# jeremy-rifkin/Markov-Huffman-Coding

Hardware: AMD Instinct MI355X
Metric: encode+decode GB/s on 16 GB byte stream, bit-exact round-trip (higher is better)
Workload: dtype u8

## Files before the change

markov-huffman-coding_amd/csrc/mh_encode.hip:

```cpp
#include "mh_dev.hpp"

namespace mhk {


constexpr uint32_t O2H_MAP_OFF = 256, O2H_HOT_OFF = 256 + 64 * 64 * 2;
__device__ __forceinline__ void o2hot_lookup16(const unsigned char *img, const uint4 &x4, uint32_t ctx, uint32_t (&e)[16]) {
    const uint16_t *ctxmap = reinterpret_cast<const uint16_t *>(img + O2H_MAP_OFF);
    const uint16_t *hot = reinterpret_cast<const uint16_t *>(img + O2H_HOT_OFF);
    const uint32_t x[4] = {x4.x, x4.y, x4.z, x4.w};
    uint32_t id[18];
    id[0] = img[ctx >> 8];
    id[1] = img[ctx & 255u];
#pragma unroll
    for (int j = 0; j < 16; ++j) id[2 + j] = img[(x[j >> 2] >> (8 * (j & 3))) & 255u];
    uint32_t cs[16];
#pragma unroll
    for (int j = 0; j < 16; ++j) cs[j] = ctxmap[(id[j] << 6) | (id[j + 1] ^ id[j])];
#pragma unroll
    for (int j = 0; j < 16; ++j) e[j] = hot[(cs[j] << 6) | (id[j + 2] ^ id[j + 1])];
}

__device__ __forceinline__ void o2hot_lookup8(const unsigned char *img, uint32_t xa, uint32_t xb, uint32_t ctx, uint32_t (&e)[8]) {
    const uint16_t *ctxmap = reinterpret_cast<const uint16_t *>(img + O2H_MAP_OFF);
    const uint16_t *hot = reinterpret_cast<const uint16_t *>(img + O2H_HOT_OFF);
// ... 533 lines not shown
                }
                if (lane == 0) {
                    const uint64_t gend = base + total;
                    __hip_atomic_store(&cp.state[group], CH_PFX | (gend & CH_VAL), __ATOMIC_RELAXED, __HIP_MEMORY_SCOPE_AGENT);
                    if ((group + 1) * E_WAVES >= p.nwt) *cp.nbits = gend;
                    if (bad) atomicExch(cp.status, MHK_STATUS_TIMEOUT);
                    s_done[par] = 0;
                    s_base[par] = base;
                    s_bad[par] = bad ? 1u : 0u;
                    __hip_atomic_store(&s_tag[par], tag, __ATOMIC_RELEASE, __HIP_MEMORY_SCOPE_WORKGROUP);
                }
            }
            uint32_t spins = 0;
            const bool follower_hook = cp.probe == 3u && group != 0 && arrived != uint32_t(E_WAVES) - 1u;
            while (__hip_atomic_load(&s_tag[par], __ATOMIC_ACQUIRE, __HIP_MEMORY_SCOPE_WORKGROUP) != tag) {
                if (++spins > CH_SPIN_MAX * 8u || follower_hook) {
                    waited_out = true;
                    if (lane == 0) atomicExch(cp.status, MHK_STATUS_TIMEOUT);
                    break;
                }
                __builtin_amdgcn_s_sleep(1);
            }
            if (follower_hook && !waited_out) {
                waited_out = true;
                if (lane == 0) atomicExch(cp.status, MHK_STATUS_TIMEOUT);
            }
            uint64_t mine = lane < wave ? s_tile[par][lane] : 0ull;
#pragma unroll
            for (int d = 8; d >= 1; d >>= 1) mine += __shfl_xor(mine, d);
            s = s_base[par] + __shfl(mine, 0);
            if (s_bad[par]) waited_out = true;
        }
        if (wt < p.nwt) {
            const uint64_t end = s + tile_bits;
            if (lane == 0 && !waited_out && end > cap_bits) atomicExch(cp.status, MHK_STATUS_CAPACITY);
            emit = !(waited_out || end > cap_bits);
        }
        if (waited_out) break;
        const uint64_t wt_now = wt;
        __syncthreads();
        if (threadIdx.x == 0) s_ticket = atomicAdd(cp.sync, 1u);
        __syncthreads();
        group = s_ticket;
        wt = group * E_WAVES + wave;
        ahead = load_raw2(p.data, p.n, wt * E_WT + lane * E_VEC, p.prev0);
        if (emit) {
            uint64_t gbase = s >> 5;
            uint32_t cur = uint32_t(s & 31u);
            uint64_t abs_bits = s;
            uint32_t seam0 = (cur != 0 && wt_now != 0) ? SEAM_DROP : SEAM_NONE;
#pragma unroll 1
            for (int k = 0; k < E_SUBSTEPS; ++k) {
                const uint64_t off = wt_now * E_WT + uint64_t(k) * E_SUB + lane * E_VEC;
                const uint32_t nvalid = off + E_VEC <= p.n ? uint32_t(E_VEC) : off < p.n ? uint32_t(p.n - off) : 0u;
                uint32_t sub_bits;
                if ((escmask >> k) & 1u) {
                    const LaneIn again = load_raw2(p.data, p.n, off, p.prev0);
                    emit_substep_slow<2>(p, nullptr, stage, out32, again.x, h0.pb, nvalid, lane, off, abs_bits, gbase, cur, seam0, sub_bits);
                } else {
                    const uint32_t L = (h0.gl & 255u) + ((h0.gl >> 8) & 255u) + ((h0.gl >> 16) & 255u) + (h0.gl >> 24);
                    const uint32_t inc = wave_inclusive_sum(L);
                    sub_bits = __builtin_amdgcn_readlane(inc, 63);
                    const uint32_t exc = inc - L;
                    if (p.index && nvalid && ((uint32_t(off) & (S - 1u)) == 0u))
                        p.index[off >> p.chunk_shift] = (uint64_t(h0.pb) << 48) | (abs_bits + exc);
                    fine2_entry(p, S, lane, off, nvalid, h0.pb, exc);
                    uint32_t o = cur + exc;
#pragma unroll
                    for (int q = 0; q < 4; ++q) {
                        const uint32_t glq = (h0.gl >> (8 * q)) & 255u;
                        if (glq) deposit<false>(stage, h0.g[q] << (64u - glq), o, 0, 0);
                        o += glq;
                    }
                    const uint32_t nfull = (cur + sub_bits) >> 5;
                    flush_words(stage, out32, gbase, nfull, seam0, lane);
                    if (nfull) seam0 = SEAM_NONE;
                    gbase += nfull;
                    cur = (cur + sub_bits) & 31u;
                }
                abs_bits += sub_bits;
                h0 = h1; h1 = h2; h2 = h3;
            }
            if (cur != 0 && seam0 == SEAM_NONE) {
                const uint64_t next = (wt_now + 1) * uint64_t(E_WT);
                const uint64_t pos = next + lane;
                const bool valid = lane < 32u && pos < p.n;
                uint32_t l = 0;
                uint64_t c = 0;
                if (valid) o2_code_of(p, smem, p.data[pos - 2], p.data[pos - 1], p.data[pos], l, c);
                const uint32_t inc = wave_inclusive_sum(l);
                const uint32_t exc = inc - l;
                if (l && exc < 32u - cur) deposit<true>(stage, c << (64u - l), cur + exc, 0u, 1u);
                if (lane == 0) {
                    out32[gbase] = __builtin_bswap32(stage[0]);
                    stage[0] = 0;
                }
            } else if (cur != 0 && lane == 0) {
                stage[0] = 0;
            }
        }
    }
}

constexpr int R_IMG_WORDS = ((163840 - 131072 - 128) / 4) & ~7;
constexpr int R_HALF_WORDS = R_IMG_WORDS / 2;
constexpr uint32_t R_HALF_CAP_BITS = uint32_t(R_HALF_WORDS - 8) * 32u;
static_assert(R_IMG_WORDS >= E_WAVES * (E_STAGE_BITS / 32) + 16 && R_HALF_WORDS % 4 == 0, "image size");
constexpr int REGION_LDS_BYTES = 131072 + R_IMG_WORDS * 4 + 128;



__global__ __launch_bounds__(1024) void region_bits_kernel(const HistHeader *hdr, HistHeader expect, const uint32_t *slab,
                                                           const uint32_t *cross_all, const uint8_t *len8,
                                                           unsigned long long *region_bits, uint32_t *region_esc, int *status) {
    __shared__ unsigned long long part[16];
    __shared__ uint32_t any_esc;
    extern __shared__ __attribute__((aligned(16))) unsigned char lens[];
    for (uint32_t i = threadIdx.x; i < 65536u / 16u; i += 1024u) reinterpret_cast<uint4 *>(lens)[i] = reinterpret_cast<const uint4 *>(len8)[i];
    if (threadIdx.x == 0) any_esc = 0;
    __syncthreads();
    const uint32_t w = blockIdx.x, tid = threadIdx.x;
    if (hdr->magic != HIST_WS_MAGIC || hdr->n != expect.n || hdr->data != expect.data || hdr->region_vecs != expect.region_vecs ||
        hdr->grid != expect.grid || hdr->prev0 != expect.prev0 || hdr->cross_cap != expect.cross_cap) {
        if (tid == 0) { atomicExch(status, MHK_STATUS_CORRUPT); region_bits[w] = 0; region_esc[w] = 0; }
        return;
    }
    unsigned long long acc = 0;
    bool esc = false;
    const uint32_t *sl = slab + size_t(w) * 32768u;
    for (uint32_t i = tid; i < 32768u; i += 1024u) {
        const uint32_t v = sl[i];
        const uint32_t s0 = i, s1 = i | 0x8000u;
        const uint32_t l0 = lens[hist_slot_prev(s0) * 256u + (s0 >> 8)], l1 = lens[hist_slot_prev(s1) * 256u + (s1 >> 8)];
        acc += (unsigned long long)(v & 0xFFFFu) * l0;
        acc += (unsigned long long)(v >> 16) * l1;
        esc |= ((v & 0xFFFFu) && l0 > uint32_t(mh::ENC16_MAX_LEN)) || ((v >> 16) && l1 > uint32_t(mh::ENC16_MAX_LEN));
    }
    const uint32_t *cross = cross_all + size_t(w) * (expect.cross_cap + 1u);
    const uint32_t nc = cross[0];
    if (nc > expect.cross_cap && tid == 0) atomicExch(status, MHK_STATUS_CAPACITY);
    for (uint32_t i = tid; i < (nc < expect.cross_cap ? nc : expect.cross_cap); i += 1024u) {
        const uint32_t sl2 = cross[1u + i];
        const uint32_t l2 = lens[hist_slot_prev(sl2) * 256u + (sl2 >> 8)];
        acc += 16384ull * l2;
        esc |= l2 > uint32_t(mh::ENC16_MAX_LEN);
    }
    if (esc) atomicOr(&any_esc, 1u);
    for (int d = 32; d >= 1; d >>= 1) acc += __shfl_xor(acc, d);
    if ((tid & 63u) == 0) part[tid >> 6] = acc;
    __syncthreads();
    if (tid == 0) {
        unsigned long long t = 0;
        for (int i = 0; i < 16; ++i) t += part[i];
        region_bits[w] = t;
        region_esc[w] = any_esc;
    }
}

__global__ __launch_bounds__(SCAN_THREADS) void region_scan_kernel(const unsigned long long *region_bits, uint32_t nregion,
                                                                   unsigned long long *region_start, const unsigned long long *carry0,
                                                                   uint8_t *out, uint64_t cap, unsigned long long *nbits, int *status) {
    __shared__ uint64_t lds[SCAN_THREADS / 64];
    const uint64_t c0 = carry0 ? (*carry0 & 7ull) : 0;
    const uint32_t i = threadIdx.x;
    const uint64_t v = i < nregion ? region_bits[i] : 0;
    uint64_t total;
    const uint64_t ex = block_excl_scan(v, lds, total);
    const uint64_t s = c0 + ex;
    if (i < nregion) {
        region_start[i] = s;
        if (i > 0 && (s & 31u) && ((s >> 5) + 1) * 4 <= cap) reinterpret_cast<uint32_t *>(out)[s >> 5] = 0;
    }
    if (i == 0) {
        const uint64_t end = c0 + total;
        *nbits = end;
        if (end > cap * 8) atomicExch(status, MHK_STATUS_CAPACITY);
        const uint64_t endw = end >> 5;
        if ((end & 31u) && (endw + 1) * 4 <= cap) reinterpret_cast<uint32_t *>(out)[endw] = 0;
        else if (end & 31u) for (uint64_t b = endw * 4; b < cap; ++b) out[b] = 0;
        if ((c0 & 31u) && 4 <= cap) reinterpret_cast<uint32_t *>(out)[0] = 0;
    }
}

struct RegionParams {
    const unsigned long long *region_start;
    const unsigned long long *region_bits;
    const uint32_t *region_esc;
    uint64_t region_vecs;
    uint64_t nvec_up;
    uint64_t cap_words;
    int *status;
};
constexpr uint32_t R_IMG_CAP_BITS = E_WAVES * E_STAGE_BITS;

struct Roll1 {
    uint4 x; uint32_t prev;
    __device__ __forceinline__ uint32_t next_window() {
        const uint32_t sym = x.x & 255u;
        const uint32_t win = (sym << 8) | prev;
        prev = sym;
        x.x = __builtin_amdgcn_alignbyte(x.y, x.x, 1);
        x.y = __builtin_amdgcn_alignbyte(x.z, x.y, 1);
        x.z = __builtin_amdgcn_alignbyte(x.w, x.z, 1);
        x.w >>= 8;
        return win;
    }
};
__device__ __forceinline__ void code_of1(const uint8_t *len8, const uint64_t *code64, const uint16_t *tab, uint32_t win, bool valid, uint32_t &l, uint64_t &c) {
    const uint32_t e = valid ? uint32_t(tab[mh::enc_slot(win)]) : 0u;
    l = e >> 12;
    c = e & 0xFFFu;
    if (e >= 0xD000u) {
        const uint32_t nat = ((win & 255u) << 8) | (win >> 8);
        l = len8[nat];
        c = code64[nat];
        if (l > 64u) { l = 0; c = 0; }
    }
}
__device__ __forceinline__ uint32_t region_escape_bits(const uint8_t *len8, const uint64_t *code64, const uint16_t *tab, uint4 x, uint32_t pb, uint32_t nvalid) {
    Roll1 r{x, pb};
    uint32_t L = 0;
#pragma unroll 1
    for (uint32_t j = 0; j < 16; ++j) { uint32_t l; uint64_t c; code_of1(len8, code64, tab, r.next_window(), j < nvalid, l, c); L += l; }
    return L;
}
__device__ __forceinline__ void region_escape_deposit(const uint8_t *len8, const uint64_t *code64, const uint16_t *tab, uint32_t *img, uint4 x,
                                                   uint32_t pb, uint32_t nvalid, uint32_t o) {
    Roll1 r{x, pb};
#pragma unroll 1
    for (uint32_t j = 0; j < 16; ++j) {
        uint32_t l; uint64_t c;
        code_of1(len8, code64, tab, r.next_window(), j < nvalid, l, c);
        if (l) deposit<false>(img, c << (64u - l), o, 0, 0);
        o += l;
    }
}

__device__ __forceinline__ uint32_t region_round_lanes(uint64_t nsym, uint64_t bits) {
    const uint32_t cand[4] = {1024u, 1008u, 992u, 960u};
    uint32_t pick = 0;
#pragma unroll
    for (int c = 3; c >= 0; --c)
        if (bits * cand[c] * E_VEC * 201u <= uint64_t(R_HALF_CAP_BITS - 32u) * nsym * 200u) pick = cand[c];
    return pick ? pick : 1024u;
}

#ifdef MH_ENC_STAMP
#define ENC_STAMP(i) do { unsigned long long t_; __builtin_amdgcn_sched_barrier(0); \
        asm volatile("s_memtime %0\n\ts_waitcnt lgkmcnt(0)" : "=s"(t_) :: "memory"); __builtin_amdgcn_sched_barrier(0); \
        stamp_acc[i] += t_ - stamp_last; stamp_last = t_; } while (0)
#else
#define ENC_STAMP(i) do { } while (0)
#endif
template <bool ESCK, bool WIDE = false>
__global__ __launch_bounds__(E_THREADS) void enc_region_kernel(EmitParams p, RegionParams rp) {
    extern __shared__ __attribute__((aligned(16))) unsigned char smem[];
    if ((rp.region_esc[blockIdx.x] != 0) != ESCK) return;
    {
        const uint64_t v0 = uint64_t(blockIdx.x) * rp.region_vecs;
        const uint64_t v1 = v0 + rp.region_vecs < rp.nvec_up ? v0 + rp.region_vecs : rp.nvec_up;
        if (v0 < v1) {
            const uint32_t rs = ESCK ? uint32_t(E_THREADS) : region_round_lanes((v1 * E_VEC < p.n ? v1 * E_VEC : p.n) - v0 * E_VEC, rp.region_bits[blockIdx.x]);
            if ((rs != uint32_t(E_THREADS)) != WIDE) return;
        } else if (WIDE) return;
    }
    uint16_t *tab = reinterpret_cast<uint16_t *>(smem);
    uint32_t *img = reinterpret_cast<uint32_t *>(smem + 131072);
    uint32_t *sb = img + R_IMG_WORDS;
    const uint32_t tid = threadIdx.x, lane = tid & 63u, wave = tid >> 6;
    for (int i = tid; i < 8192; i += E_THREADS)
        reinterpret_cast<uint4 *>(tab)[i] = reinterpret_cast<const uint4 *>(p.enc16)[i];
    for (int i = tid; i < R_IMG_WORDS; i += E_THREADS) img[i] = 0;
    __syncthreads();
    if (*p.status != MHK_STATUS_OK) return;

    const uint64_t v0 = uint64_t(blockIdx.x) * rp.region_vecs;
    const uint64_t v1 = v0 + rp.region_vecs < rp.nvec_up ? v0 + rp.region_vecs : rp.nvec_up;
    if (v0 >= v1) return;
    uint32_t *out32 = reinterpret_cast<uint32_t *>(p.out);
    const uint32_t S = 1u << p.chunk_shift;
    const uint32_t RS = WIDE ? region_round_lanes((v1 * E_VEC < p.n ? v1 * E_VEC : p.n) - v0 * E_VEC, rp.region_bits[blockIdx.x]) : uint32_t(E_THREADS);
    const bool act = !WIDE || tid < RS;
    const bool wave_idles = WIDE && uint32_t(wave) * 64u + 63u >= RS;
    const uint64_t rounds = (v1 - v0 + RS - 1) / RS;
    const uint64_t s0 = rp.region_start[blockIdx.x];
    uint64_t gbase = s0 >> 5, abs_round = s0;
    uint32_t cur = uint32_t(s0 & 31u);
    bool seam_first = cur != 0;
    uint32_t carry = 0;
    bool prev_half = false;

    auto fetch = [&](uint64_t r) -> LaneIn {
        const uint64_t v = v0 + r * RS + tid;
        LaneIn in = load_raw(p.data, p.n, (act && v < v1) ? v * E_VEC : ~0ull >> 1, p.prev0);
        return in;
    };
    auto lookup16 = [&](const LaneIn &in, uint32_t pb, uint32_t (&e)[16]) {
        uint32_t w[16];
        slots16(in.x, pb, w);
#pragma unroll
        for (int j = 0; j < 16; ++j) e[j] = uint32_t(tab[w[j]]);
    };
    uint32_t *imgr = img;
    auto flush = [&](uint32_t nfull) -> uint32_t {
        uint32_t tail = 0;
        for (uint32_t j = tid * 4u; j <= nfull; j += E_THREADS * 4u) {
            const uint4 w = *reinterpret_cast<const uint4 *>(imgr + j);
            *reinterpret_cast<uint4 *>(imgr + j) = make_uint4(0, 0, 0, 0);
            const uint32_t v[4] = {__builtin_bswap32(w.x), __builtin_bswap32(w.y), __builtin_bswap32(w.z), __builtin_bswap32(w.w)};
            if (j + 4u <= nfull && !(j == 0 && seam_first) && gbase + j + 4u <= rp.cap_words) {
                struct __attribute__((packed, aligned(4))) Q4 { uint32_t a, b, c, d; };
                *reinterpret_cast<Q4 *>(out32 + gbase + j) = Q4{v[0], v[1], v[2], v[3]};
            } else {
#pragma unroll
                for (uint32_t k = 0; k < 4u; ++k) {
                    if (j + k >= nfull || gbase + j + k >= rp.cap_words) break;
                    if (j + k == 0 && seam_first) atomicOr(&out32[gbase], v[k]);
                    else out32[gbase + j + k] = v[k];
                }
            }
            if (nfull - j < 4u) {
                const uint32_t k = nfull - j;
                tail = k == 0 ? w.x : k == 1 ? w.y : k == 2 ? w.z : w.w;
            }
        }
        return tail;
    };
#ifdef MH_ENC_STAMP
    unsigned long long stamp_acc[6] = {0, 0, 0, 0, 0, 0}, stamp_last = 0;
    asm volatile("s_memtime %0\n\ts_waitcnt lgkmcnt(0)" : "=s"(stamp_last) :: "memory");
#endif
    struct Packed { uint64_t g[4]; uint32_t gl[4]; uint32_t L, inc; bool esc; };
    auto pack = [&](const uint32_t (&E)[16], const LaneIn &in, uint32_t pb, auto full_c, auto esc_c) __attribute__((always_inline)) -> Packed {
        constexpr bool FULL = decltype(full_c)::value, ESC = decltype(esc_c)::value;
        Packed P;
        uint32_t e[16];
#pragma unroll
        for (int j = 0; j < 16; ++j) e[j] = (FULL || uint32_t(j) < in.nvalid) ? E[j] : 0u;
        if (FULL && wave_idles) {
#pragma unroll
            for (int j = 0; j < 16; ++j) e[j] = act ? e[j] : 0u;
        }
        P.L = 0;
        uint32_t emax = 0;
#pragma unroll
        for (int q = 0; q < 4; ++q) {
            const uint32_t e0 = e[4 * q], e1 = e[4 * q + 1], e2 = e[4 * q + 2], e3 = e[4 * q + 3];
            if (ESC) {
                const uint32_t m01 = e0 > e1 ? e0 : e1, m23 = e2 > e3 ? e2 : e3;
                emax = emax > m01 ? emax : m01;
                emax = emax > m23 ? emax : m23;
            }
            const uint32_t l0 = e0 >> 12, l1 = e1 >> 12, l2 = e2 >> 12, l3 = e3 >> 12;
            const uint32_t p01 = ((e0 & 0xFFFu) << l1) | (e1 & 0xFFFu);
            const uint32_t p23 = ((e2 & 0xFFFu) << l3) | (e3 & 0xFFFu);
            P.g[q] = (uint64_t(p01) << (l2 + l3)) | p23;
            P.gl[q] = l0 + l1 + l2 + l3;
            P.L += P.gl[q];
        }
        P.esc = ESC && emax >= 0xD000u;
        if (ESC && __any(P.esc)) {
            if (P.esc) P.L = region_escape_bits(p.len8, p.code64, tab, in.x, pb, FULL ? uint32_t(E_VEC) : in.nvalid);
        }
        P.inc = wave_inclusive_sum(P.L);
        return P;
    };
    auto fetch_full = [&](uint64_t r) -> LaneIn {
        LaneIn in;
        const uint64_t v = v0 + r * RS + tid;
        in.x = reinterpret_cast<const uint4 *>(p.data)[v];
        in.nvalid = act ? uint32_t(E_VEC) : 0u;
        in.head = p.prev0;
        if (lane == 0 && v) in.head = uint32_t(p.data[v * E_VEC - 1]);
        return in;
    };
    using ESC_T = std::integral_constant<bool, ESCK>;
    LaneIn D0 = fetch(0), D1 = fetch(1), D2 = fetch(2), D3 = fetch(3);
    uint32_t pb0 = head_byte(D0), pb1 = head_byte(D1);
    uint32_t E1[16];
    Packed P;
    {
        uint32_t E0[16];
        lookup16(D0, pb0, E0);
        lookup16(D1, pb1, E1);
        P = pack(E0, D0, pb0, std::false_type{}, ESC_T{});
    }
    if (lane == 63) sb[wave] = P.inc;
    uint4 x0 = D0.x;
    uint32_t nvalid0 = D0.nvalid;
    static_assert(E_WAVES == 16, "the scan below is one DPP row");
    auto round = [&](uint64_t r, auto full_c, uint32_t (&Ea)[16], uint32_t (&Eb)[16]) __attribute__((always_inline)) {
        constexpr bool FULL = decltype(full_c)::value, ESC = ESCK;
        uint32_t *sbr = sb + (r & 1u) * 16u, *sbn = sb + ((r + 1u) & 1u) * 16u;
        ENC_STAMP(0);
        uint32_t cs = sbr[lane & 15u];
        if (r == 0 || !prev_half) { __syncthreads(); cs = sbr[lane & 15u]; }
        ENC_STAMP(1);
        cs += uint32_t(__builtin_amdgcn_update_dpp(0, int(cs), 0x111, 0xF, 0xF, true));
        cs += uint32_t(__builtin_amdgcn_update_dpp(0, int(cs), 0x112, 0xF, 0xF, true));
        cs += uint32_t(__builtin_amdgcn_update_dpp(0, int(cs), 0x114, 0xF, 0xF, true));
        cs += uint32_t(__builtin_amdgcn_update_dpp(0, int(cs), 0x118, 0xF, 0xF, true));
        const uint32_t tot = uint32_t(__builtin_amdgcn_readlane(int(cs), 15));
        const uint32_t pre = wave ? uint32_t(__builtin_amdgcn_readlane(int(cs), int(wave) - 1)) : 0u;
        const bool half = !ESC && cur + tot <= R_HALF_CAP_BITS;
        if (!half && r != 0 && prev_half) __syncthreads();
        imgr = half ? img + (r & 1u) * uint32_t(R_HALF_WORDS) : img;
        prev_half = half;
        if (carry) { atomicOr(&imgr[0], carry); carry = 0; }
        const uint32_t exc = pre + P.inc - P.L;
        const uint64_t off = (v0 + r * RS + tid) * E_VEC;
        const uint32_t nvalid = FULL ? (act ? uint32_t(E_VEC) : 0u) : nvalid0;
        if (p.index && nvalid && ((uint32_t(off) & (S - 1u)) == 0u))
            p.index[off >> p.chunk_shift] = (uint64_t(pb0) << 56) | (abs_round + exc);
        if (p.fine && nvalid && (lane & (uint32_t(1u << T_SUB_SHIFT) / 16u - 1u)) == 0u)
            p.fine[off >> T_SUB_SHIFT] = (pb0 << 24) | (uint32_t(abs_round + exc) & FINE_POS_MASK);
        const bool fits = !ESC || cur + tot <= R_IMG_CAP_BITS;
        if (fits) {
            uint32_t o = cur + exc;
            if (!ESC || !P.esc) {
#pragma unroll
                for (int q = 0; q < 4; ++q) {
                    if (P.gl[q]) deposit<false>(imgr, P.g[q] << (64u - P.gl[q]), o, 0, 0);
                    o += P.gl[q];
                }
            } else {
                region_escape_deposit(p.len8, p.code64, tab, imgr, x0, pb0, nvalid, o);
            }
        } else {
            for (uint32_t m = 0; m < uint32_t(E_WAVES); ++m) {
                const uint32_t upto = uint32_t(__builtin_amdgcn_readlane(int(cs), int(m)));
                const uint32_t before = m ? uint32_t(__builtin_amdgcn_readlane(int(cs), int(m) - 1)) : 0u;
                if (wave == m) region_escape_deposit(p.len8, p.code64, tab, img, x0, pb0, nvalid, cur + (exc - pre));
                __syncthreads();
                const uint32_t nfull = (cur + (upto - before)) >> 5;
                const uint32_t t = flush(nfull);
                seam_first = seam_first && nfull == 0;
                gbase += nfull;
                cur = (cur + (upto - before)) & 31u;
                __syncthreads();
                if (t) atomicOr(&img[0], t);
            }
        }
        ENC_STAMP(2);
        const LaneIn D4 = FULL ? fetch_full(r + 4) : fetch(r + 4);
        const uint32_t pb2 = head_byte(D2);
        lookup16(D2, pb2, Eb);
        const Packed Pn = pack(Ea, D1, pb1, full_c, ESC_T{});
        if (lane == 63) sbn[wave] = Pn.inc;
        ENC_STAMP(3);
        if (fits) {
            __syncthreads();
            ENC_STAMP(4);
            const uint32_t nfull = (cur + tot) >> 5;
            carry = flush(nfull);
            seam_first = seam_first && nfull == 0;
            gbase += nfull;
            cur = (cur + tot) & 31u;
        }
        abs_round += tot;
        P = Pn;
        x0 = D1.x; nvalid0 = D1.nvalid; pb0 = pb1;
        D1 = D2; pb1 = pb2;
        D2 = D3;
        D3 = D4;
    };
    const uint64_t whole = (p.n >> 4) < v1 ? (p.n >> 4) : v1;
    const uint64_t rounds_full = whole > v0 + (E_THREADS - RS) ? (whole - v0 - (E_THREADS - RS)) / RS : 0;
    const uint64_t r_fast = rounds_full > 4 ? rounds_full - 4 : 0;
    uint64_t r = 0;
    uint32_t E2[16];
#pragma unroll 1
    for (; r + 1 < r_fast; r += 2) {
        round(r, std::true_type{}, E1, E2);
        round(r + 1, std::true_type{}, E2, E1);
    }
#pragma unroll 1
    for (; r < rounds; ++r) {
        round(r, std::false_type{}, E1, E2);
#pragma unroll
        for (int j = 0; j < 16; ++j) E1[j] = E2[j];
    }
    if (cur != 0 && gbase < rp.cap_words) {
        if (carry) atomicOr(&out32[gbase], __builtin_bswap32(carry));
        else if (tid == 0 && img[0]) atomicOr(&out32[gbase], __builtin_bswap32(img[0]));
    }
    if (tid == 0 && abs_round != s0 + rp.region_bits[blockIdx.x]) atomicExch(rp.status, MHK_STATUS_CORRUPT);
#ifdef MH_ENC_STAMP
    if (lane == 0)
        for (int i = 0; i < 5; ++i) atomicAdd(reinterpret_cast<unsigned long long *>(rp.status) + 1 + i, stamp_acc[i]);
#endif
}


__global__ __launch_bounds__(E_THREADS) void enc2_len_kernel(LenParams p) {
    const uint32_t lane = threadIdx.x & 63u;
    const uint64_t wave0 = uint64_t(blockIdx.x) * E_WAVES + (threadIdx.x >> 6);
    const uint64_t nwaves = uint64_t(gridDim.x) * E_WAVES;
    for (uint64_t wt = wave0; wt < p.nwt; wt += nwaves) {
        uint32_t sum = 0;
#pragma unroll 1
        for (int k = 0; k < E_SUBSTEPS; ++k) {
            const LaneIn in = load_raw2(p.data, p.n, wt * E_WT + uint64_t(k) * E_SUB + lane * E_VEC, p.prev0);
            uint32_t ctx = head_ctx(in);
            const uint32_t x[4] = {in.x.x, in.x.y, in.x.z, in.x.w};
            uint32_t l[16];
#pragma unroll
            for (int j = 0; j < 16; ++j) {
                const uint32_t key = (ctx << 8) | ((x[j >> 2] >> (8 * (j & 3))) & 255u);
                l[j] = uint32_t(j) < in.nvalid ? uint32_t(p.len_slot[key]) : 0u;
                ctx = key & 0xFFFFu;
            }
#pragma unroll
            for (int j = 0; j < 16; ++j) sum += l[j] > 64u ? 0u : l[j];
        }
        sum = wave_sum(sum);
        if (lane == 0) p.wt_bits[wt] = sum;
    }
}

__global__ __launch_bounds__(E_THREADS) void enc2_emit_kernel(EmitParams p) {
    extern __shared__ __attribute__((aligned(16))) unsigned char smem[];
    const uint32_t lane = threadIdx.x & 63u, wave = threadIdx.x >> 6;
    uint32_t *stage = reinterpret_cast<uint32_t *>(smem) + wave * E_STAGE_WORDS;
    for (int i = lane; i < E_STAGE_WORDS; i += 64) stage[i] = 0;
    __syncthreads();
    if (*p.status != MHK_STATUS_OK) return;
    uint32_t *out32 = reinterpret_cast<uint32_t *>(p.out);
    const uint64_t wave0 = uint64_t(blockIdx.x) * E_WAVES + wave;
    const uint64_t nwaves = uint64_t(gridDim.x) * E_WAVES;
    for (uint64_t wt = wave0; wt < p.nwt; wt += nwaves) {
        const uint64_t s = p.wt_start[wt];
        uint64_t gbase = s >> 5;
        uint32_t cur = uint32_t(s & 31u);
        uint64_t abs_bits = s;
        uint32_t seam0 = cur != 0 ? SEAM_OR : SEAM_NONE;
#pragma unroll 1
        for (int k = 0; k < E_SUBSTEPS; ++k) {
            const uint64_t off = wt * E_WT + uint64_t(k) * E_SUB + lane * E_VEC;
            const LaneIn in = load_raw2(p.data, p.n, off, p.prev0);
            const uint32_t ctx0 = head_ctx(in);
            uint32_t l[16];
            uint64_t c[16];
            const uint32_t x[4] = {in.x.x, in.x.y, in.x.z, in.x.w};
            bool escape = p.enc64 == nullptr;
            if (p.enc64) {
                uint32_t ctx = ctx0;
#pragma unroll
                for (int j = 0; j < 16; ++j) {
                    const uint32_t key = (ctx << 8) | ((x[j >> 2] >> (8 * (j & 3))) & 255u);
                    const uint64_t e = uint32_t(j) < in.nvalid ? p.enc64[key] : 0ull;
                    l[j] = uint32_t(e >> 56);
                    c[j] = e & 0x00FFFFFFFFFFFFFFull;
                    escape = escape || l[j] == 255u;
                    ctx = key & 0xFFFFu;
                }
            }
            if (__any(escape)) {
                uint32_t ctx = ctx0;
#pragma unroll
                for (int j = 0; j < 16; ++j) {
                    const uint32_t key = (ctx << 8) | ((x[j >> 2] >> (8 * (j & 3))) & 255u);
                    const bool valid = uint32_t(j) < in.nvalid;
                    l[j] = valid ? uint32_t(p.len8[key]) : 0u;
                    c[j] = valid ? p.code64[key] : 0ull;
                    ctx = key & 0xFFFFu;
                }
            }
            uint32_t L = 0;
#pragma unroll
            for (int j = 0; j < 16; ++j) { if (l[j] > 64u) l[j] = 0; L += l[j]; }
            const uint32_t inc = wave_inclusive_sum(L);
            uint32_t sub_bits = __builtin_amdgcn_readlane(inc, 63);
            if (cur + sub_bits <= uint32_t(E_STAGE_WORDS - 3) * 32u) {
                const uint32_t exc = inc - L;
                const uint32_t S = 1u << p.chunk_shift;
                if (p.index && in.nvalid && ((uint32_t(off) & (S - 1u)) == 0u))
                    p.index[off >> p.chunk_shift] = (uint64_t(ctx0) << 48) | (abs_bits + exc);
                fine2_entry(p, S, lane, off, in.nvalid, ctx0, exc);
                uint32_t o = cur + exc;
#pragma unroll
                for (int j = 0; j < 16; ++j) {
                    if (l[j]) deposit<false>(stage, c[j] << (64u - l[j]), o, 0, 0);
                    o += l[j];
                }
                const uint32_t nfull = (cur + sub_bits) >> 5;
                flush_words(stage, out32, gbase, nfull, seam0, lane);
                if (nfull) seam0 = SEAM_NONE;
                gbase += nfull;
                cur = (cur + sub_bits) & 31u;
            } else {
                emit_substep_slow<2>(p, nullptr, stage, out32, in.x, ctx0, in.nvalid, lane, off, abs_bits, gbase, cur, seam0, sub_bits);
            }
            abs_bits += sub_bits;
        }
        if (cur != 0 && lane == 0) {
            atomicOr(&out32[gbase], __builtin_bswap32(stage[0]));
            stage[0] = 0;
        }
    }
}

uint64_t encode_wave_tiles(uint64_t n) { return (n + E_WT - 1) / E_WT; }

struct EncWs { size_t off_bits, off_start, off_blk, total; uint64_t nwt, nblk; };
static EncWs enc_ws_layout(uint64_t n) {
    EncWs w;
    w.nwt = encode_wave_tiles(n);
    w.nblk = (w.nwt + SCAN_BLOCK - 1) / SCAN_BLOCK;
    auto up = [](size_t v) { return (v + 63) & ~size_t(63); };
    w.off_bits = 64;
    w.off_start = up(w.off_bits + size_t(w.nwt) * 4);
    w.off_blk = up(w.off_start + size_t(w.nwt) * 8);
    w.total = up(w.off_blk + size_t(w.nblk + 1) * 8);
    if (w.total < 64 + 2 * 1024 * 8 + 1024 * 4) w.total = 64 + 2 * 1024 * 8 + 1024 * 4;
    return w;
}
size_t encode_workspace_bytes(uint64_t n) { return enc_ws_layout(n).total; }

__global__ void empty_payload_kernel(const unsigned long long *start_bit, unsigned long long *nbits, uint8_t *out, uint64_t cap) {
    const unsigned long long b0 = start_bit ? (*start_bit & 7ull) : 0;
    *nbits = b0;
    if (b0 && cap) out[0] = 0;
}

__global__ __launch_bounds__(256) void payload_bits_kernel(const unsigned long long *counts, const uint8_t *len8, uint32_t entries,
                                                           unsigned long long *out) {
    __shared__ unsigned long long part[256];
    unsigned long long acc = 0;
    for (uint32_t i = blockIdx.x * 256u + threadIdx.x; i < entries; i += gridDim.x * 256u) acc += counts[i] * len8[i];
    part[threadIdx.x] = acc;
    __syncthreads();
    for (int d = 128; d > 0; d >>= 1) {
        if (int(threadIdx.x) < d) part[threadIdx.x] += part[threadIdx.x + d];
        __syncthreads();
    }
    if (threadIdx.x == 0 && part[0]) atomicAdd(out, part[0]);
}

hipError_t launch_payload_bits(const unsigned long long *d_counts, const uint8_t *d_len8, uint32_t entries, unsigned long long *d_out,
                               hipStream_t st) {
    hipError_t e = hipMemsetAsync(d_out, 0, 8, st);
    if (e != hipSuccess) return e;
    const unsigned grid = entries > 65536u ? 1024u : 1u;
    hipLaunchKernelGGL(payload_bits_kernel, dim3(grid), dim3(256), 0, st, d_counts, d_len8, entries, d_out);
    return hipGetLastError();
}

static bool encode2_two_pass() {
    const char *v = getenv("MH_ENCODE2_PATH");
    return v && !strcmp(v, "two_pass");
}

hipError_t launch_encode(const EncodeArgs &a, void *d_ws, hipStream_t st) {
    unsigned char *ws = static_cast<unsigned char *>(d_ws);
    const EncWs L = enc_ws_layout(a.n);
    int *status = reinterpret_cast<int *>(ws);
    hipError_t e = hipMemsetAsync(ws, 0, 64, st);
    if (e != hipSuccess) return e;
    if (a.n == 0) {
        hipLaunchKernelGGL(empty_payload_kernel, dim3(1), dim3(1), 0, st, a.start_bit, a.nbits, a.out, a.cap);
        return hipGetLastError();
    }
    e = once_per_device(&DeviceState::encode_ready, [] {
        hipError_t r = allow_lds(reinterpret_cast<const void *>(enc_len_kernel<1>), LEN_LDS_BYTES);
        if (r == hipSuccess) r = allow_lds(reinterpret_cast<const void *>(enc_len_kernel<2>), LEN_LDS_BYTES);
        if (r == hipSuccess) r = allow_lds(reinterpret_cast<const void *>(enc_emit_kernel<2>), EMIT_LDS_BYTES);
        return r != hipSuccess ? r : allow_lds(reinterpret_cast<const void *>(enc_emit_kernel<1>), EMIT_LDS_BYTES);
    });
    if (e != hipSuccess) return e;
    (void)launch_set_word(reinterpret_cast<uint32_t *>(ws + 8), uint32_t(ENC_PATH_LENGTH_PASS), st);
    uint32_t *wt_bits = reinterpret_cast<uint32_t *>(ws + L.off_bits);
    unsigned long long *wt_start = reinterpret_cast<unsigned long long *>(ws + L.off_start);
    unsigned long long *blk_sum = reinterpret_cast<unsigned long long *>(ws + L.off_blk);

    uint64_t want = (L.nwt + E_WAVES - 1) / E_WAVES;
    int grid = int(want > uint64_t(2 * cu_count()) ? uint64_t(2 * cu_count()) : want);
    const bool hot2 = a.order == 2 && a.o2hot && a.o2hot_bytes && a.o2hot_bytes <= uint32_t(LEN_LDS_BYTES);
    if (hot2 && !a.no_chain && !encode2_two_pass()) {
        e = once_per_device(&DeviceState::chain_ready, [] { return allow_lds(reinterpret_cast<const void *>(enc_chain_kernel), EMIT_LDS_BYTES); });
        if (e != hipSuccess) return e;
        const uint64_t groups = (L.nwt + E_WAVES - 1) / E_WAVES;
        e = hipMemsetAsync(wt_start, 0, size_t(groups) * 8, st);
        if (e != hipSuccess) return e;
        (void)launch_set_word(reinterpret_cast<uint32_t *>(ws + 8), uint32_t(ENC_PATH_CHAIN), st);
        ChainParams cp;
        cp.e = EmitParams{a.data, a.n, a.prev0, a.chunk_shift, a.out, a.enc16, a.len8, a.code64, a.enc64, nullptr, L.nwt, a.index, status,
                          a.fine, a.o2hot, a.o2hot_bytes};
        cp.state = wt_start;
        cp.start_bit = a.start_bit;
        cp.cap = a.cap & ~uint64_t(3);
        cp.nbits = a.nbits;
        cp.status = status;
        const char *probe = getenv("MH_CHAIN_PROBE");
        cp.probe = !probe ? 0u : !strcmp(probe, "timeout") ? 2u : !strcmp(probe, "timeout_follower") ? 3u : 0u;
#ifdef MH_EXP_PROBES
        if (probe && !strcmp(probe, "nolookback")) cp.probe = 1u;
#endif
        cp.sync = reinterpret_cast<uint32_t *>(ws + 32);
        const int cgrid = int(groups > uint64_t(cu_count()) ? uint64_t(cu_count()) : groups);
        hipLaunchKernelGGL(enc_chain_kernel, dim3(cgrid), dim3(E_THREADS), ((a.o2hot_bytes + 15u) & ~15u) + E_WAVES * E_STAGE_WORDS * 4, st, cp);
        return hipGetLastError();
    }
    if (hot2) {
        LenParams lp{a.data, a.n, a.prev0, a.len8, wt_bits, L.nwt, a.o2hot, a.o2hot_bytes};
        hipLaunchKernelGGL(enc_len_kernel<2>, dim3(grid), dim3(E_THREADS), (a.o2hot_bytes + 15u) & ~15u, st, lp);
    } else if (a.order == 2) {
        LenParams lp{a.data, a.n, a.prev0, a.len8, wt_bits, L.nwt, nullptr, 0};
        hipLaunchKernelGGL(enc2_len_kernel, dim3(grid), dim3(E_THREADS), 0, st, lp);
    } else {
        LenParams lp{a.data, a.n, a.prev0, a.len_slot, wt_bits, L.nwt, nullptr, 0};
        hipLaunchKernelGGL(enc_len_kernel<1>, dim3(grid), dim3(E_THREADS), LEN_LDS_BYTES, st, lp);
    }

    hipLaunchKernelGGL(scan_local_kernel, dim3(unsigned(L.nblk)), dim3(SCAN_THREADS), 0, st, wt_bits, L.nwt, wt_start, blk_sum);
    hipLaunchKernelGGL(scan_top_kernel, dim3(1), dim3(SCAN_THREADS), 0, st, blk_sum, L.nblk, a.start_bit);
    ScanParams sp{wt_start, blk_sum, L.nwt, L.nblk, a.out, a.cap & ~uint64_t(3), a.nbits, status};
    hipLaunchKernelGGL(scan_apply_kernel, dim3(unsigned(L.nblk)), dim3(SCAN_THREADS), 0, st, sp);

    EmitParams ep{a.data, a.n, a.prev0, a.chunk_shift, a.out, a.enc16, a.len8, a.code64, a.enc64, wt_start, L.nwt, a.index, status,
                  a.fine, a.o2hot, a.o2hot_bytes};
    if (hot2) {
        grid = int(want > uint64_t(cu_count()) ? uint64_t(cu_count()) : want);
        hipLaunchKernelGGL(enc_emit_kernel<2>, dim3(grid), dim3(E_THREADS), ((a.o2hot_bytes + 15u) & ~15u) + E_WAVES * E_STAGE_WORDS * 4, st, ep);
        return hipGetLastError();
    }
    if (a.order == 2) {
        hipLaunchKernelGGL(enc2_emit_kernel, dim3(grid), dim3(E_THREADS), E_WAVES * E_STAGE_WORDS * 4, st, ep);
        return hipGetLastError();
    }
    grid = int(want > uint64_t(cu_count()) ? uint64_t(cu_count()) : want);
    hipLaunchKernelGGL(enc_emit_kernel<1>, dim3(grid), dim3(E_THREADS), EMIT_LDS_BYTES, st, ep);
    return hipGetLastError();
}

hipError_t launch_encode_regions(const EncodeArgs &a, const void *d_hist_ws, size_t hist_ws_bytes, void *d_ws, hipStream_t st) {
    unsigned char *ws = static_cast<unsigned char *>(d_ws);
    int *status = reinterpret_cast<int *>(ws);
    hipError_t e = hipMemsetAsync(ws, 0, 64, st);
    if (e != hipSuccess) return e;
    if (a.n == 0) {
        hipLaunchKernelGGL(empty_payload_kernel, dim3(1), dim3(1), 0, st, a.start_bit, a.nbits, a.out, a.cap);
        return hipGetLastError();
    }
    const RegionGeom g = region_geom(a.n);
    if (!d_hist_ws || hist_ws_bytes < g.total || g.grid > 1024) return hipErrorInvalidValue;
    e = once_per_device(&DeviceState::region_ready, [] {
        hipError_t r = allow_lds(reinterpret_cast<const void *>(enc_region_kernel<false>), REGION_LDS_BYTES);
        if (r == hipSuccess) r = allow_lds(reinterpret_cast<const void *>(enc_region_kernel<false, true>), REGION_LDS_BYTES);
        if (r == hipSuccess) r = allow_lds(reinterpret_cast<const void *>(region_bits_kernel), 65536);
        return r != hipSuccess ? r : allow_lds(reinterpret_cast<const void *>(enc_region_kernel<true>), REGION_LDS_BYTES);
    });
    if (e != hipSuccess) return e;
    const unsigned char *hws = static_cast<const unsigned char *>(d_hist_ws);
    unsigned long long *region_bits = reinterpret_cast<unsigned long long *>(ws + 64);
    unsigned long long *region_start = region_bits + 1024;
    uint32_t *region_esc = reinterpret_cast<uint32_t *>(region_start + 1024);
    const HistHeader expect{HIST_WS_MAGIC, a.n, reinterpret_cast<unsigned long long>(a.data), g.region_vecs, uint32_t(g.grid), a.prev0, g.cross_cap, 0};
    hipLaunchKernelGGL(region_bits_kernel, dim3(g.grid), dim3(1024), 65536, st, reinterpret_cast<const HistHeader *>(hws + 64), expect,
                       reinterpret_cast<const uint32_t *>(hws + g.off_slab), reinterpret_cast<const uint32_t *>(hws + g.off_cross), a.len8,
                       region_bits, region_esc, status);
    hipLaunchKernelGGL(region_scan_kernel, dim3(1), dim3(SCAN_THREADS), 0, st, region_bits, uint32_t(g.grid), region_start, a.start_bit,
                       a.out, a.cap & ~uint64_t(3), a.nbits, status);
    EmitParams ep{a.data, a.n, a.prev0, a.chunk_shift, a.out, a.enc16, a.len8, a.code64, nullptr, nullptr, 0, a.index, status, a.fine, nullptr, 0};
    RegionParams rp{region_start, region_bits, region_esc, g.region_vecs, g.nvec_up, (a.cap & ~uint64_t(3)) >> 2, status};
    (void)launch_set_word(reinterpret_cast<uint32_t *>(ws + 8), uint32_t(a.max_len > mh::ENC16_MAX_LEN ? ENC_PATH_REGIONS_ESCAPES : ENC_PATH_REGIONS), st);
    hipLaunchKernelGGL(enc_region_kernel<false>, dim3(g.grid), dim3(E_THREADS), REGION_LDS_BYTES, st, ep, rp);
    if (a.max_len >= 8)
        hipLaunchKernelGGL((enc_region_kernel<false, true>), dim3(g.grid), dim3(E_THREADS), REGION_LDS_BYTES, st, ep, rp);
    if (a.max_len > mh::ENC16_MAX_LEN)
        hipLaunchKernelGGL(enc_region_kernel<true>, dim3(g.grid), dim3(E_THREADS), REGION_LDS_BYTES, st, ep, rp);
    return hipGetLastError();
}

__global__ __launch_bounds__(256) void enc64_pack_kernel(const uint8_t *len8, const unsigned long long *code64, unsigned long long *enc64, uint64_t n) {
    for (uint64_t i = uint64_t(blockIdx.x) * 256 + threadIdx.x; i < n; i += uint64_t(gridDim.x) * 256) {
        const uint32_t l = len8[i];
        enc64[i] = l <= 56u ? ((unsigned long long)(l) << 56) | code64[i] : 0xFF00000000000000ull;
    }
}
hipError_t launch_enc64_pack(const uint8_t *len8, const uint64_t *code64, uint64_t *enc64, uint64_t n, hipStream_t st) {
    hipLaunchKernelGGL(enc64_pack_kernel, dim3(unsigned(cu_count()) * 8u), dim3(256), 0, st, len8,
                       reinterpret_cast<const unsigned long long *>(code64), reinterpret_cast<unsigned long long *>(enc64), n);
    return hipGetLastError();
}
// ... 14 lines not shown
```

Measured before the change: 561.6.

## Interleave table lookups, deposits and flush with the block-wide prefix scan

Restructures the encoder round so the next vector's code-table lookups are split into four groups. These groups are interleaved with the current round's flush stores, the bit deposits (now done inside pack, per quad) and the shared-memory prefix-scan read, which is precomputed into cs_pre right after the barrier. Lookup results are kept as a 16-bit array, and sched_barrier fences force this ordering. The goal is to hide LDS/global lookup latency behind the store and scan work and to reduce register pressure. In exchange the compiler's freedom to schedule is constrained, and the ordering logic becomes more complex.

```diff
diff --git a/markov-huffman-coding_amd/csrc/mh_encode.hip b/markov-huffman-coding_amd/csrc/mh_encode.hip
--- a/markov-huffman-coding_amd/csrc/mh_encode.hip
+++ b/markov-huffman-coding_amd/csrc/mh_encode.hip
@@ -859,28 +859,42 @@
         for (int j = 0; j < 16; ++j) e[j] = uint32_t(tab[w[j]]);
     };
     uint32_t *imgr = img;
+    auto flush_take = [&](uint32_t j, uint32_t nfull) -> uint4 {
+        uint4 w = make_uint4(0, 0, 0, 0);
+        if (j <= nfull) {
+            w = *reinterpret_cast<const uint4 *>(imgr + j);
+            *reinterpret_cast<uint4 *>(imgr + j) = make_uint4(0, 0, 0, 0);
+        }
+        return w;
+    };
+    auto flush_store = [&](uint32_t j, uint32_t nfull, const uint4 &w, uint32_t &tail) {
+        const uint32_t v[4] = {__builtin_bswap32(w.x), __builtin_bswap32(w.y), __builtin_bswap32(w.z), __builtin_bswap32(w.w)};
+        if (j > nfull) return;
+        if (j + 4u <= nfull && !(j == 0 && seam_first) && gbase + j + 4u <= rp.cap_words) {
+            struct __attribute__((packed, aligned(4))) Q4 { uint32_t a, b, c, d; };
+            *reinterpret_cast<Q4 *>(out32 + gbase + j) = Q4{v[0], v[1], v[2], v[3]};
+        } else {
+#pragma unroll
+            for (uint32_t k = 0; k < 4u; ++k) {
+                if (j + k >= nfull || gbase + j + k >= rp.cap_words) break;
+                if (j + k == 0 && seam_first) atomicOr(&out32[gbase], v[k]);
+                else out32[gbase + j + k] = v[k];
+            }
+        }
+        if (nfull - j < 4u) {
+            const uint32_t k = nfull - j;
+            tail = k == 0 ? w.x : k == 1 ? w.y : k == 2 ? w.z : w.w;
+        }
+    };
+    auto flush_from = [&](uint32_t j, uint32_t nfull, uint32_t &tail) {
+        for (; j <= nfull; j += E_THREADS * 4u) {
+            const uint4 w = flush_take(j, nfull);
+            flush_store(j, nfull, w, tail);
+        }
+    };
     auto flush = [&](uint32_t nfull) -> uint32_t {
         uint32_t tail = 0;
-        for (uint32_t j = tid * 4u; j <= nfull; j += E_THREADS * 4u) {
-            const uint4 w = *reinterpret_cast<const uint4 *>(imgr + j);
-            *reinterpret_cast<uint4 *>(imgr + j) = make_uint4(0, 0, 0, 0);
-            const uint32_t v[4] = {__builtin_bswap32(w.x), __builtin_bswap32(w.y), __builtin_bswap32(w.z), __builtin_bswap32(w.w)};
-            if (j + 4u <= nfull && !(j == 0 && seam_first) && gbase + j + 4u <= rp.cap_words) {
-                struct __attribute__((packed, aligned(4))) Q4 { uint32_t a, b, c, d; };
-                *reinterpret_cast<Q4 *>(out32 + gbase + j) = Q4{v[0], v[1], v[2], v[3]};
-            } else {
-#pragma unroll
-                for (uint32_t k = 0; k < 4u; ++k) {
-                    if (j + k >= nfull || gbase + j + k >= rp.cap_words) break;
-                    if (j + k == 0 && seam_first) atomicOr(&out32[gbase], v[k]);
-                    else out32[gbase + j + k] = v[k];
-                }
-            }
-            if (nfull - j < 4u) {
-                const uint32_t k = nfull - j;
-                tail = k == 0 ? w.x : k == 1 ? w.y : k == 2 ? w.z : w.w;
-            }
-        }
+        flush_from(tid * 4u, nfull, tail);
         return tail;
     };
 #ifdef MH_ENC_STAMP
@@ -888,21 +902,22 @@
     asm volatile("s_memtime %0\n\ts_waitcnt lgkmcnt(0)" : "=s"(stamp_last) :: "memory");
 #endif
     struct Packed { uint64_t g[4]; uint32_t gl[4]; uint32_t L, inc; bool esc; };
-    auto pack = [&](const uint32_t (&E)[16], const LaneIn &in, uint32_t pb, auto full_c, auto esc_c) __attribute__((always_inline)) -> Packed {
+    auto pack = [&](const auto (&E)[16], const LaneIn &in, uint32_t pb, auto full_c, auto esc_c, auto before) __attribute__((always_inline)) -> Packed {
         constexpr bool FULL = decltype(full_c)::value, ESC = decltype(esc_c)::value;
         Packed P;
-        uint32_t e[16];
-#pragma unroll
-        for (int j = 0; j < 16; ++j) e[j] = (FULL || uint32_t(j) < in.nvalid) ? E[j] : 0u;
-        if (FULL && wave_idles) {
-#pragma unroll
-            for (int j = 0; j < 16; ++j) e[j] = act ? e[j] : 0u;
-        }
         P.L = 0;
         uint32_t emax = 0;
 #pragma unroll
         for (int q = 0; q < 4; ++q) {
-            const uint32_t e0 = e[4 * q], e1 = e[4 * q + 1], e2 = e[4 * q + 2], e3 = e[4 * q + 3];
+            before(q);
+            uint32_t e[4];
+#pragma unroll
+            for (int j = 0; j < 4; ++j) e[j] = (FULL || uint32_t(4 * q + j) < in.nvalid) ? uint32_t(E[4 * q + j]) : 0u;
+            if (FULL && wave_idles) {
+#pragma unroll
+                for (int j = 0; j < 4; ++j) e[j] = act ? e[j] : 0u;
+            }
+            const uint32_t e0 = e[0], e1 = e[1], e2 = e[2], e3 = e[3];
             if (ESC) {
                 const uint32_t m01 = e0 > e1 ? e0 : e1, m23 = e2 > e3 ? e2 : e3;
                 emax = emax > m01 ? emax : m01;
@@ -913,6 +928,7 @@
             const uint32_t p23 = ((e2 & 0xFFFu) << l3) | (e3 & 0xFFFu);
             P.g[q] = (uint64_t(p01) << (l2 + l3)) | p23;
             P.gl[q] = l0 + l1 + l2 + l3;
+            asm volatile("" : "+v"(P.g[q]), "+v"(P.gl[q]));
             P.L += P.gl[q];
         }
         P.esc = ESC && emax >= 0xD000u;
@@ -934,31 +950,46 @@
     using ESC_T = std::integral_constant<bool, ESCK>;
     LaneIn D0 = fetch(0), D1 = fetch(1), D2 = fetch(2), D3 = fetch(3);
     uint32_t pb0 = head_byte(D0), pb1 = head_byte(D1);
-    uint32_t E1[16];
+    uint32_t W[16];
+    uint16_t E[16];
+    auto look4 = [&](int g) __attribute__((always_inline)) {
+#pragma unroll
+        for (int j = 4 * g; j < 4 * g + 4; ++j) E[j] = tab[W[j]];
+    };
+    const auto nothing = [](int) {};
     Packed P;
     {
         uint32_t E0[16];
         lookup16(D0, pb0, E0);
-        lookup16(D1, pb1, E1);
-        P = pack(E0, D0, pb0, std::false_type{}, ESC_T{});
-    }
+        P = pack(E0, D0, pb0, std::false_type{}, ESC_T{}, nothing);
+    }
+    slots16(D1.x, pb1, W);
+    look4(0); look4(1); look4(2);
     if (lane == 63) sb[wave] = P.inc;
     uint4 x0 = D0.x;
     uint32_t nvalid0 = D0.nvalid;
+    uint32_t cs_pre = 0;
     static_assert(E_WAVES == 16, "the scan below is one DPP row");
-    auto round = [&](uint64_t r, auto full_c, uint32_t (&Ea)[16], uint32_t (&Eb)[16]) __attribute__((always_inline)) {
-        constexpr bool FULL = decltype(full_c)::value, ESC = ESCK;
-        uint32_t *sbr = sb + (r & 1u) * 16u, *sbn = sb + ((r + 1u) & 1u) * 16u;
-        ENC_STAMP(0);
-        uint32_t cs = sbr[lane & 15u];
-        if (r == 0 || !prev_half) { __syncthreads(); cs = sbr[lane & 15u]; }
-        ENC_STAMP(1);
+    auto row_scan16 = [](uint32_t cs) __attribute__((always_inline)) -> uint32_t {
         cs += uint32_t(__builtin_amdgcn_update_dpp(0, int(cs), 0x111, 0xF, 0xF, true));
         cs += uint32_t(__builtin_amdgcn_update_dpp(0, int(cs), 0x112, 0xF, 0xF, true));
         cs += uint32_t(__builtin_amdgcn_update_dpp(0, int(cs), 0x114, 0xF, 0xF, true));
         cs += uint32_t(__builtin_amdgcn_update_dpp(0, int(cs), 0x118, 0xF, 0xF, true));
+        return cs;
+    };
+    auto round = [&](uint64_t r, auto full_c) __attribute__((always_inline)) {
+        constexpr bool FULL = decltype(full_c)::value, ESC = ESCK;
+        uint32_t *sbr = sb + (r & 1u) * 16u, *sbn = sb + ((r + 1u) & 1u) * 16u;
+        ENC_STAMP(0);
+        uint32_t cs = cs_pre;
+        if (r == 0 || !prev_half) { __syncthreads(); cs = row_scan16(sbr[lane & 15u]); }
+        ENC_STAMP(1);
         const uint32_t tot = uint32_t(__builtin_amdgcn_readlane(int(cs), 15));
         const uint32_t pre = wave ? uint32_t(__builtin_amdgcn_readlane(int(cs), int(wave) - 1)) : 0u;
+        __builtin_amdgcn_sched_barrier(0);
+        look4(3);
+        const uint32_t pb2 = head_byte(D2);
+        __builtin_amdgcn_sched_barrier(0);
         const bool half = !ESC && cur + tot <= R_HALF_CAP_BITS;
         if (!half && r != 0 && prev_half) __syncthreads();
         imgr = half ? img + (r & 1u) * uint32_t(R_HALF_WORDS) : img;
@@ -972,18 +1003,7 @@
         if (p.fine && nvalid && (lane & (uint32_t(1u << T_SUB_SHIFT) / 16u - 1u)) == 0u)
             p.fine[off >> T_SUB_SHIFT] = (pb0 << 24) | (uint32_t(abs_round + exc) & FINE_POS_MASK);
         const bool fits = !ESC || cur + tot <= R_IMG_CAP_BITS;
-        if (fits) {
-            uint32_t o = cur + exc;
-            if (!ESC || !P.esc) {
-#pragma unroll
-                for (int q = 0; q < 4; ++q) {
-                    if (P.gl[q]) deposit<false>(imgr, P.g[q] << (64u - P.gl[q]), o, 0, 0);
-                    o += P.gl[q];
-                }
-            } else {
-                region_escape_deposit(p.len8, p.code64, tab, imgr, x0, pb0, nvalid, o);
-            }
-        } else {
+        if (!fits) {
             for (uint32_t m = 0; m < uint32_t(E_WAVES); ++m) {
                 const uint32_t upto = uint32_t(__builtin_amdgcn_readlane(int(cs), int(m)));
                 const uint32_t before = m ? uint32_t(__builtin_amdgcn_readlane(int(cs), int(m) - 1)) : 0u;
@@ -998,21 +1018,43 @@
                 if (t) atomicOr(&img[0], t);
             }
         }
+        uint32_t o = cur + exc;
+        const bool dep = fits && (!ESC || !P.esc);
+        const Packed Pn = pack(E, D1, pb1, full_c, ESC_T{}, [&](int q) __attribute__((always_inline)) {
+            if (dep && P.gl[q]) deposit<false>(imgr, P.g[q] << (64u - P.gl[q]), o, 0, 0);
+            o += P.gl[q];
+        });
+        if (ESC && fits && P.esc) region_escape_deposit(p.len8, p.code64, tab, imgr, x0, pb0, nvalid, cur + exc);
+        if (lane == 63) sbn[wave] = Pn.inc;
         ENC_STAMP(2);
         const LaneIn D4 = FULL ? fetch_full(r + 4) : fetch(r + 4);
-        const uint32_t pb2 = head_byte(D2);
-        lookup16(D2, pb2, Eb);
-        const Packed Pn = pack(Ea, D1, pb1, full_c, ESC_T{});
-        if (lane == 63) sbn[wave] = Pn.inc;
+        slots16(D2.x, pb2, W);
         ENC_STAMP(3);
         if (fits) {
             __syncthreads();
             ENC_STAMP(4);
             const uint32_t nfull = (cur + tot) >> 5;
-            carry = flush(nfull);
+            const uint32_t j0 = tid * 4u;
+            uint32_t tail = 0;
+            const uint4 w = flush_take(j0, nfull);
+            cs_pre = sbn[lane & 15u];
+            look4(0);
+            __builtin_amdgcn_sched_barrier(0);
+            flush_store(j0, nfull, w, tail);
+            __builtin_amdgcn_sched_barrier(0);
+            look4(1);
+            __builtin_amdgcn_sched_barrier(0);
+            flush_from(j0 + E_THREADS * 4u, nfull, tail);
+            carry = tail;
             seam_first = seam_first && nfull == 0;
             gbase += nfull;
             cur = (cur + tot) & 31u;
+            __builtin_amdgcn_sched_barrier(0);
+            look4(2);
+            __builtin_amdgcn_sched_barrier(0);
+            cs_pre = row_scan16(cs_pre);
+        } else {
+            look4(0); look4(1); look4(2);
         }
         abs_round += tot;
         P = Pn;
@@ -1025,18 +1067,13 @@
     const uint64_t rounds_full = whole > v0 + (E_THREADS - RS) ? (whole - v0 - (E_THREADS - RS)) / RS : 0;
     const uint64_t r_fast = rounds_full > 4 ? rounds_full - 4 : 0;
     uint64_t r = 0;
-    uint32_t E2[16];
 #pragma unroll 1
     for (; r + 1 < r_fast; r += 2) {
-        round(r, std::true_type{}, E1, E2);
-        round(r + 1, std::true_type{}, E2, E1);
+        round(r, std::true_type{});
+        round(r + 1, std::true_type{});
     }
 #pragma unroll 1
-    for (; r < rounds; ++r) {
-        round(r, std::false_type{}, E1, E2);
-#pragma unroll
-        for (int j = 0; j < 16; ++j) E1[j] = E2[j];
-    }
+    for (; r < rounds; ++r) round(r, std::false_type{});
     if (cur != 0 && gbase < rp.cap_words) {
         if (carry) atomicOr(&out32[gbase], __builtin_bswap32(carry));
         else if (tid == 0 && img[0]) atomicOr(&out32[gbase], __builtin_bswap32(img[0]));
```

After: 566.6 (median of 6 runs). Within noise of the previous version (+0.9%).
